# huangjh-pub/di-fusion

Hardware: AMD Instinct MI355X
Metric: frames/s integrate+decode+mesh, 640x480 synthetic stream (higher is better)
Workload: dtype f32

## Files before the change

### di_fusion_amd/_lib.py

```python
from __future__ import annotations

import ctypes
import os
from ctypes import POINTER, Structure, c_float, c_int32, c_int64, c_uint8, c_void_p
from pathlib import Path

PKG = Path(__file__).resolve().parent
LIB_PATH = Path(os.environ["DIF_LIB"]) if os.environ.get("DIF_LIB") else PKG / "libdifusion.so"

C_N_OCCUPIED, C_OVERFLOW, C_ALLOC_NEW, C_M, C_C, C_ITEMS, C_K, C_B, C_VH, C_T, C_QUERY_M, C_N_KEPT, C_CACHE_T, C_CACHE_KEPT, C_EXPORT_N, C_WORK, C_CACHE_DEAD, C_CACHE_LIVE, C_OPT_ROWS, C_OPT_VOXELS, C_HALO_L, C_HALO_R, C_HALO_TICKET, C_DEFERRED = range(24)
C_ALLOC_KEPT = 24
C_STAMP = 31
SYNC_FUSED, SYNC_FRONT_DONE, SYNC_WORDS = 0, 32, 64
FC_COUNT = 32
C_COUNT = 32
PROF_NAMES = ["encode", "decode_lattice", "decode_points", "mc_count", "mc_emit", "halo_export", "halo_merge"]
PROF_COUNT = 8
LATENT_DIM = 29

ERRORS = {-1: "DIF_EINVAL (bad argument)", -2: "DIF_ELAUNCH (HIP launch/runtime failure)", -3: "DIF_ENOSPACE (workspace too small)"}


class DifMap(Structure):
    _fields_ = [("nx", c_int32), ("ny", c_int32), ("nz", c_int32),
# ... 178 lines not shown
    "dif_marching_cubes": (c_int32, [c_void_p, c_int32, c_int32, c_int32, c_void_p, c_int64, c_void_p, c_int64, c_void_p,
                                     c_void_p, c_int32, c_float, c_int64, c_void_p, c_void_p, c_void_p, c_void_p,
                                     c_void_p, c_void_p, c_void_p, c_void_p]),
    "dif_decode_rows": (c_int32, [POINTER(DifWeights), c_void_p, c_int64, c_void_p, c_void_p, c_void_p]),
    "dif_encode_rows": (c_int32, [POINTER(DifWeights), c_void_p, c_int64, c_void_p, c_void_p]),
    "dif_query_sdf": (c_int32, [POINTER(DifMap), POINTER(DifWeights), c_void_p, c_int64, c_void_p, c_void_p, c_void_p,
                                c_void_p, c_void_p, c_void_p, c_void_p]),
    "dif_query_select": (c_int32, [POINTER(DifMap), c_void_p, c_int64, c_void_p, c_void_p, c_void_p, c_void_p, c_int32, c_void_p]),
    "dif_query_decode": (c_int32, [POINTER(DifMap), POINTER(DifWeights), c_void_p, c_int64, c_void_p, c_void_p, c_void_p, c_void_p, c_void_p]),
    "dif_query_grad_scatter": (c_int32, [c_void_p, c_void_p, c_void_p, c_int64, c_void_p, c_void_p]),
    "dif_query_grad_gather": (c_int32, [c_void_p, c_void_p, c_void_p, c_int64, c_void_p, c_void_p]),
    "dif_export_records": (c_int32, [POINTER(DifMap), c_void_p, c_int64, c_int32, c_int32, c_int32, c_void_p, c_void_p]),
    "dif_merge_records": (c_int32, [POINTER(DifMap), c_void_p, c_int64, c_int32, c_void_p, c_void_p]),
    "dif_export_halo": (c_int32, [POINTER(DifMap), c_void_p, c_int64, c_int32, c_int32, c_void_p, c_void_p]),
    "dif_merge_halo": (c_int32, [POINTER(DifMap), c_void_p, c_int64, c_void_p, c_void_p]),
    "dif_export_halo_delta": (c_int32, [POINTER(DifMap), c_void_p, c_void_p, c_int64, c_void_p, c_void_p]),
    "dif_halo_lists_reset": (c_int32, [POINTER(DifMap), c_void_p, c_void_p, c_void_p, c_void_p]),
    "dif_merge_halo2": (c_int32, [POINTER(DifMap), c_void_p, c_int64, c_void_p, c_int64, c_void_p, c_void_p, c_void_p]),
    "dif_profile_enable": (c_int32, [c_int32]),
    "dif_profile_read": (c_int32, [POINTER(ctypes.c_double), POINTER(c_int64), c_int32]),
    "dif_profile_dump": (c_int64, [POINTER(c_int32), POINTER(c_float), c_int64, c_int32]),
    "dif_read_counters": (c_int32, [POINTER(DifMap), POINTER(c_int32), c_void_p]),
    "dif_test_mc_grid_cap": (c_int32, [c_int32]),
    "dif_test_sdma_mode": (c_int32, [c_int32]),
    "dif_test_optimize_views": (c_int32, [c_int64, c_int64, c_void_p, POINTER(DifOptimizeViews)]),
    "dif_test_integrate_views": (c_int32, [c_int64, c_void_p, POINTER(DifIntegrateViews)]),
    "dif_test_sdf_hg_views": (c_int32, [c_int64, c_void_p, POINTER(DifSdfHgViews)]),
    "dif_test_sdf_hg_reduce": (c_int32, [c_void_p, c_int64, POINTER(DifSdfHg), c_void_p, c_int64, c_void_p, c_void_p]),
    "dif_sdma_info": (c_int32, [POINTER(c_int32)]),
    "dif_test_handoff": (c_int32, [c_int32, c_int32, c_int32, c_int32, POINTER(c_int64)]),
    "dif_queues_independent": (c_int32, [c_void_p, c_void_p]),
    "dif_mesh_cache_export_sdma": (c_int32, [POINTER(DifExtractBuffers), c_int64, c_int64, c_void_p, c_void_p, c_void_p]),
    "dif_sdf_hg_workspace_bytes": (c_int64, [c_int64]),
    "dif_sdf_hg": (c_int32, [POINTER(DifMap), POINTER(DifWeights), c_void_p, c_int64, POINTER(DifSdfHg), c_void_p, c_int64, c_void_p, c_void_p,
                             c_int64, c_void_p]),
    "dif_gradient_xy": (c_int32, [c_void_p, c_int32, c_int32, c_void_p, c_void_p]),
    "dif_photo_pyramid": (c_int32, [c_void_p, c_void_p, c_int32, c_int32, POINTER(DifPhotoPyramid), c_void_p]),
    "dif_rgb_odometry": (c_int32, [c_void_p, c_void_p, c_void_p, c_void_p, c_void_p, c_int32, c_int32, POINTER(DifRgbHg), c_void_p, c_void_p,
                                   c_void_p]),
    "dif_rgb_hg_workspace_bytes": (c_int64, []),
    "dif_rgb_hg": (c_int32, [c_void_p, c_void_p, c_void_p, c_void_p, c_void_p, c_int32, c_int32, POINTER(DifRgbHg), c_void_p, c_int64, c_void_p,
                             c_void_p, c_int64, c_void_p]),
}

_lib = None

# ... 63 lines not shown
```

### di_fusion_amd/csrc/difusion.hip

```cpp
#include <cstdlib>
#include <cstdio>
#include <cstring>
#include <mutex>
#include <atomic>
#include <chrono>
#include <vector>
#include <hip/hip_runtime.h>
#include <hsa/hsa.h>
#include <hsa/hsa_ext_amd.h>
#include <dlfcn.h>

#include "common.hip.h"
#include "mlp.hip.h"
#include "mc_tables.inc"

using namespace dif;

namespace {

constexpr int L = DIF_LATENT_DIM;

__device__ __constant__ int c_mc_edge_table[256];
__device__ __constant__ unsigned long long c_mc_tri_packed[256];
bool g_tables_uploaded[64] = {};
// ... 838 lines not shown

struct ExtractGeo { int r, R, l, R3; double sample_a, sample_b; };
static ExtractGeo extract_geo(int resolution) {
    ExtractGeo e;
    e.r = resolution; e.R = 2 * resolution; e.l = resolution;
    e.R3 = e.R * e.R * e.R;
    e.sample_a = -(double)(e.r / 2) * (1.0 / e.r);
    e.sample_b = 1.0 + (double)((e.r - 1) / 2) * (1.0 / e.r);
    return e;
}

static DirtySet dirty_set_of(const dif_map_t* map, const dif_extract_buffers_t* buf, int no_cache) {
    const int64_t grid = (int64_t)map->nx * map->ny * map->nz, plane = (int64_t)map->ny * map->nz;
    const bool tiled = map_is_tiled(map);
    const int64_t own_lo = tiled ? map->own_x_lo * plane : 0, own_hi = tiled ? map->own_x_hi * plane : grid;
    return DirtySet{map->dirty, map->latent_vecs_pos, buf->valid_blocks, map->counters, no_cache, buf->max_voxels, geo_of(map), map->ignore_count_th,
                    map->indexer, map->voxel_obs_count, grid_marks_of(map), own_lo, own_hi, tiled};
}

static VoxelDecodeArgs voxel_decode_args_of(const dif_map_t* map, const dif_weights_t* w, const dif_extract_buffers_t* buf, const ExtractGeo& e, bool fold) {
    VoxelDecodeArgs V = {};
    V.occ_slot = buf->occ_slot; V.latent = map->latent_vecs; V.cube_sdf = buf->cube_sdf; V.cube_std = buf->cube_std;
    V.counters = map->counters;
    V.refine_list = buf->refine_list; V.R = e.R;
    V.fold_w = fold ? w->dec_fold_packed : nullptr; V.fold_table = buf->fold_table;
    V.low.res = e.l; V.low.a = (float)e.sample_a; V.low.vsize = (e.l > 1) ? (float)((e.sample_b - e.sample_a) / (e.l - 1)) : 0.0f;
    return V;
}

static DecodeArgs refine_args_of(const dif_map_t* map, const dif_extract_buffers_t* buf, const ExtractGeo& e, bool fold) {
    DecodeArgs Rf = {};
    Rf.mode = 1; Rf.n_ptr = map->counters + DIF_C_VH; Rf.occ_slot = buf->occ_slot; Rf.latent = map->latent_vecs; Rf.list = buf->refine_list;
    Rf.lat.res = e.R; Rf.lat.a = (float)e.sample_a; Rf.lat.vsize = (float)((e.sample_b - e.sample_a) / (e.R - 1));
    Rf.fold_table = fold ? buf->fold_table : nullptr;
    Rf.out_sdf = buf->cube_sdf; Rf.out_std = buf->cube_std; Rf.sign = -1.0f;
    return Rf;
}

static McArgs mc_args_of(const dif_map_t* map, const dif_extract_buffers_t* buf, const ExtractGeo& e, float max_std, int scale_vertices) {
    int* C = map->counters;
    McArgs a = {};
    a.indexer = map->indexer; a.nx = map->nx; a.ny = map->ny; a.nz = map->nz; a.valid_blocks = buf->valid_blocks; a.K_ptr = C + DIF_C_K; a.K_static = 0;
    a.vbm = map->vbm; a.V = map->capacity; a.cube_sdf = buf->cube_sdf; a.cube_std = buf->cube_std; a.R = e.R; a.max_std = max_std;
    a.max_triangles = buf->cache_capacity; a.new_limit = buf->max_triangles; a.base_ptr = C + DIF_C_CACHE_KEPT;
    a.triangles = buf->cache_tri; a.tri_id = buf->cache_id; a.tri_std = buf->cache_std; a.tri_alive = buf->cache_alive;
    a.scale = scale_vertices ? 1 : 0; a.vs = map->voxel_size; a.bx = map->bound_min[0]; a.by = map->bound_min[1]; a.bz = map->bound_min[2];
    a.log_counters = C;
// ... 24 lines not shown
                                 defer ? (dif_pending_export_t*)map->pending_export : nullptr, buf->stamp, defer ? buf->export_notify : nullptr},
                      (fused_scan && !onepass) ? buf->chunk_sum : nullptr, super_sum, map->dirty_tot, (int)((map->capacity + DIF_BLOCK - 1) / DIF_BLOCK),
                      onepass ? buf->mc_status : nullptr, onepass ? buf->mc_status + (buf->max_voxels + 3) / 4 : nullptr,
                      ov ? map->frame_counters : nullptr};
}

constexpr size_t VD_LDS_F32 = ((size_t)((DEC_LDS_FLOATS + 3) & ~3) + 4 * VD_WAVE_LDS_FLOATS) * 4, VD_LDS_X6 = (size_t)X6_LDS_BYTES + 4 * VD_WAVE_LDS_FLOATS * 4;
static int voxel_decode_attributes() {
    static bool attr_set[64] = {};
    int dev = 0; (void)hipGetDevice(&dev);
    if (dev < 64 && !attr_set[dev]) {
        if (hipFuncSetAttribute((const void*)k_decode_voxels<false>, hipFuncAttributeMaxDynamicSharedMemorySize, (int)VD_LDS_F32) != hipSuccess) return DIF_ELAUNCH;
        if (hipFuncSetAttribute((const void*)k_decode_voxels<true>, hipFuncAttributeMaxDynamicSharedMemorySize, (int)VD_LDS_X6) != hipSuccess) return DIF_ELAUNCH;
        if (hipFuncSetAttribute((const void*)k_decode_refine_x6, hipFuncAttributeMaxDynamicSharedMemorySize, (int)X6_LDS_BYTES) != hipSuccess) return DIF_ELAUNCH;
        if (hipFuncSetAttribute((const void*)k_decode_voxels_batch<true>, hipFuncAttributeMaxDynamicSharedMemorySize, (int)VD_LDS_X6) != hipSuccess) return DIF_ELAUNCH;
        if (hipFuncSetAttribute((const void*)k_decode_refine_x6_batch, hipFuncAttributeMaxDynamicSharedMemorySize, (int)X6_LDS_BYTES) != hipSuccess) return DIF_ELAUNCH;
        attr_set[dev] = true;
    }
    return DIF_OK;
}

static std::atomic<int> g_mc_grid_cap{0};
int dif_test_mc_grid_cap(int32_t n) { return g_mc_grid_cap.exchange(n > 0 ? n : 0); }

static int mc_onepass_setup(const McArgs& a, size_t& lds_bytes, int& grid1, int64_t max_voxels) {
    if (upload_tables() != DIF_OK) return DIF_ELAUNCH;
    const int r = a.R / 2, nc = (r + 1) * (r + 1) * (r + 1);
    lds_bytes = (size_t)(DIF_BLOCK / 64) * MC_ONEPASS_WAVE_LDS_FLOATS(nc) * sizeof(float);
    if (lds_bytes > 128 * 1024) return DIF_EINVAL;
    static bool attr_set1[64] = {};
    int dev = 0; (void)hipGetDevice(&dev);
    if (dev < 64 && !attr_set1[dev]) {
        if (hipFuncSetAttribute((const void*)k_marching_cubes_onepass<0>, hipFuncAttributeMaxDynamicSharedMemorySize, 128 * 1024) != hipSuccess) return DIF_ELAUNCH;
        if (hipFuncSetAttribute((const void*)k_marching_cubes_onepass<4>, hipFuncAttributeMaxDynamicSharedMemorySize, 128 * 1024) != hipSuccess) return DIF_ELAUNCH;
        if (hipFuncSetAttribute((const void*)k_marching_cubes_onepass_batch<0>, hipFuncAttributeMaxDynamicSharedMemorySize, 128 * 1024) != hipSuccess) return DIF_ELAUNCH;
        if (hipFuncSetAttribute((const void*)k_marching_cubes_onepass_batch<4>, hipFuncAttributeMaxDynamicSharedMemorySize, 128 * 1024) != hipSuccess) return DIF_ELAUNCH;
        attr_set1[dev] = true;
    }
    const int64_t need = (max_voxels + 3) / 4;
    int per_cu = (int)((160 * 1024) / (lds_bytes + 1024));
    per_cu = per_cu < 1 ? 1 : per_cu > MC_WAVES_PER_SIMD ? MC_WAVES_PER_SIMD : per_cu;
    grid1 = per_cu * num_cus();
    if (need < grid1) grid1 = (int)(need < 1 ? 1 : need);
    { const int n = g_mc_grid_cap.load(std::memory_order_relaxed); if (n > 0 && n < grid1) grid1 = n; }
    return DIF_OK;
}
// ... 49 lines not shown
    const bool totals = map->dirty_tot && !no_cache && !P.dirty.tiled;
    P.scan = !totals ? DirtyScan::Generic : (map->capacity > 4096 && map->capacity % DIF_BLOCK == 0) ? DirtyScan::BlockTotals : DirtyScan::BoundedTotals;
    if (ov && P.scan != DirtyScan::BlockTotals) return DIF_EINVAL;
    P.fused_word = ov ? map->sync_words + DIF_SYNC_FUSED : nullptr;
    P.grid = (int64_t)map->nx * map->ny * map->nz;
    P.occ = OccFunctor{map->grid_bits, map->indexer, buf->occ_slot, map->vbm, map->counters, max_voxels};

    if (!has_dec(w)) return DIF_EINVAL;
    const bool fused = fast && e.l * e.l * e.l <= VD_MAX_L3 && e.R * e.R <= VD_MAX_R2;
    const bool fold = fused && has_dec_fold(w) && buf->fold_table;
    P.decode = !fast ? DecodeChain::Exact : !fused ? DecodeChain::TwoLevel : (fold && has_dec_x6(w)) ? DecodeChain::FusedX6 : DecodeChain::FusedF32;
    P.refine_tiles = max_voxels * (int64_t)(e.R3 / 32);
    if (P.decode == DecodeChain::Exact) {
        P.lattice = exact_lattice_args_of(map, buf, e);
        P.lattice_tiles = max_voxels * (int64_t)((e.R3 + 31) / 32);
    } else if (P.decode == DecodeChain::TwoLevel) {
        P.lattice = low_lattice_args_of(map, buf, e);
        P.lattice_tiles = max_voxels * ((e.l * e.l * e.l + 31) / 32);
        P.refine = refine_args_of(map, buf, e, false);
    } else {
        P.vd = voxel_decode_args_of(map, w, buf, e, fold);
        if (voxel_decode_attributes() != DIF_OK) return DIF_ELAUNCH;
        P.vd_lds = P.decode == DecodeChain::FusedX6 ? VD_LDS_X6 : VD_LDS_F32;
        P.vd_blocks = cu_blocks(max_voxels, 4);
        P.refine = refine_args_of(map, buf, e, fold);
        P.refine_blocks = cu_blocks(P.refine_tiles, 8);
    }

    P.mc_args = mc_args_of(map, buf, e, max_std, scale_vertices);
    const bool chunked = buf->chunk_sum && max_voxels <= ((int64_t)1 << 24);
    P.mc = !chunked ? McChain::CountScanEmit : (buf->mc_status && e.r * e.r * e.r <= 64) ? McChain::OnePass : McChain::CountEmit;
    int rc = DIF_OK;
    if (P.mc == McChain::OnePass) {
        mc_onepass_args(P.mc_args, map, buf, defer);
        rc = mc_onepass_setup(P.mc_args, P.mc_lds, P.mc_grid, max_voxels);
    } else if (P.mc == McChain::CountEmit) {
        McArgs& a = P.mc_args;
        a.chunk_sum = buf->chunk_sum; a.super_sum = buf->chunk_sum + (max_voxels + 255) / 256; a.tri_start = map->tri_start; a.tri_n = map->tri_n;
        a.tri_count = buf->tri_count; a.tri_offset = nullptr;
        rc = mc_setup(a, P.mc_lds, P.mc_grid, max_voxels);
    }
    if (rc != DIF_OK) return rc;
    P.finish = finish_args_of(map, buf, chunked, P.mc == McChain::OnePass, P.mc_args.out_tri != nullptr, defer);
    P.finish_grid = grid_for(max_voxels, DIF_BLOCK, 256);
    return DIF_OK;
}

// ... 83 lines not shown
    hipStream_t s = (hipStream_t)stream_;
    static thread_local Batch<DirtyScanArgs> dirty; static thread_local ScanBatch<OccFunctor> occ; static thread_local Batch<VoxelDecodeArgs> vd;
    static thread_local Batch<DecodeArgs> rf; static thread_local Batch<McStream> mc; static thread_local Batch<FinishArgs> fin;
    ExtractPlan P;
    for (int j = 0; j < S; ++j) {
        const int rc = extract_plan(st[j].map, w, st[j].buf, resolution, 1, max_std, 0, scale_vertices, s, P);
        if (rc != DIF_OK) return rc;
        if (P.scan != DirtyScan::BlockTotals || P.dirty.tiled || P.decode != DecodeChain::FusedX6 || P.mc != McChain::OnePass) return DIF_EINVAL;
        if (st[j].buf->max_voxels != st[0].buf->max_voxels) return DIF_EINVAL;
        dirty.s[j] = DirtyScanArgs{P.dirty, P.n_slots, st[j].map->dirty_tot};
        occ.f[j] = P.occ; occ.tot[j] = st[j].map->grid_tot;
        vd.s[j] = P.vd; rf.s[j] = P.refine;
        mc.s[j] = McStream{P.mc_args, P.finish.mc_status, P.finish.mc_ticket};
        fin.s[j] = P.finish;
    }
    for (int j = S; j < DIF_MAX_STREAMS; ++j) {
        dirty.s[j] = dirty.s[0]; occ.f[j] = occ.f[0]; occ.tot[j] = occ.tot[0]; vd.s[j] = vd.s[0]; rf.s[j] = rf.s[0]; mc.s[j] = mc.s[0]; fin.s[j] = fin.s[0];
    }
    hipLaunchKernelGGL(k_dirty_scan_batch, dim3((int)(st[0].map->capacity / DIF_BLOCK), S), dim3(DIF_BLOCK), 0, s, dirty);
    DIF_CHECK_LAUNCH();
    if (launch_counted_scan_batch(occ, S, (int)((P.grid + 31) / 32), s) != DIF_OK) return DIF_ELAUNCH;
    {
        ProfScope prof(DIF_PROF_DECODE_LATTICE, s);
        hipLaunchKernelGGL(k_decode_voxels_batch<true>, dim3(cu_blocks(P.occ.max_voxels * S, 4)), dim3(512), P.vd_lds, s, vd, (int)S, (const float*)w->dec_x6_packed);
        DIF_CHECK_LAUNCH();
    }
    {
        ProfScope prof(DIF_PROF_DECODE_POINTS, s);
        hipLaunchKernelGGL(k_decode_refine_x6_batch, dim3(cu_blocks(P.refine_tiles * S, 8)), dim3(512), (size_t)X6_LDS_BYTES, s, rf, (int)S, (const float*)w->dec_x6_packed);
        DIF_CHECK_LAUNCH();
    }
    {
        ProfScope prof(DIF_PROF_MC_COUNT, s);
        if (P.e.r == 4) hipLaunchKernelGGL(k_marching_cubes_onepass_batch<4>, dim3(P.mc_grid, S), dim3(DIF_BLOCK), P.mc_lds, s, mc);
        else hipLaunchKernelGGL(k_marching_cubes_onepass_batch<0>, dim3(P.mc_grid, S), dim3(DIF_BLOCK), P.mc_lds, s, mc);
        DIF_CHECK_LAUNCH();
    }
    hipLaunchKernelGGL(k_extract_finish_batch, dim3(P.finish_grid, S), dim3(DIF_BLOCK), 0, s, fin);
    DIF_CHECK_LAUNCH();
    return DIF_OK;
}

#ifdef DIF_TRACE
int dif_trace_read(unsigned long long* out, int64_t n) {
    return hipMemcpyFromSymbol(out, HIP_SYMBOL(g_vd_trace), (size_t)n * 8) == hipSuccess ? DIF_OK : DIF_ELAUNCH;
}
int dif_trace_read_encode(unsigned long long* out, int64_t n) {
// ... 1294 lines not shown
```

### di_fusion_amd/csrc/kernels_extract.hip.h

```cpp
#pragma once

__device__ __forceinline__ void mark_confident_nbhd(const Geo& g, int lin, float ignore_th, const int64_t* __restrict__ indexer,
                                                    const float* __restrict__ obs, const GridMarks& marks) {
    const uint32_t* bits = marks.bits;
    int ix, iy, iz;
    unlinearize(g, lin, ix, iy, iz);
    int cand[7];
    cand[0] = lin;
    cand[1] = linearize(g, clampi(ix - 1, 0, g.nx - 1), iy, iz);
    cand[2] = linearize(g, clampi(ix + 1, 0, g.nx - 1), iy, iz);
    cand[3] = linearize(g, ix, clampi(iy - 1, 0, g.ny - 1), iz);
    cand[4] = linearize(g, ix, clampi(iy + 1, 0, g.ny - 1), iz);
    cand[5] = linearize(g, ix, iy, clampi(iz - 1, 0, g.nz - 1));
    cand[6] = linearize(g, ix, iy, clampi(iz + 1, 0, g.nz - 1));
    int64_t slot[7];
#pragma unroll
    for (int c = 0; c < 7; ++c) slot[c] = indexer[cand[c]];
    float w[7];
#pragma unroll
    for (int c = 0; c < 7; ++c) w[c] = slot[c] >= 0 ? obs[slot[c]] : ignore_th;
    uint32_t word[7];
#pragma unroll
    for (int c = 0; c < 7; ++c) word[c] = (w[c] > ignore_th) ? bits[cand[c] >> 5] : 0xFFFFFFFFu;
    uint32_t prev[7];
// ... 524 lines not shown
            __syncthreads();
            int o = s_base + ex;
            while (sel) {
                int jz = __ffs((int)sel) - 1;
                sel &= sel - 1;
                refine_list[o++] = (int32_t)(e0 + jz);
            }
        }
        __syncthreads();
    }
}

struct VoxelDecodeArgs {
    const int32_t* occ_slot;
    const float* latent;
    Lattice low;
    int R;
    float* cube_sdf;
    float* cube_std;
    int32_t* refine_list;
    int* counters;
    const float* fold_w;
    float* fold_table;
};

#define VD_MAX_L3 64
#define VD_MAX_R2 64
#define VD_WAVE_LDS_FLOATS (2 * VD_MAX_L3 + 2 * 256)

#ifdef DIF_TRACE
__device__ unsigned long long g_vd_trace[2048 * 8];
#define VD_STAMP(slot) do { if (lane_id() == 0) g_vd_trace[((threadIdx.x >> 6) * gridDim.x + blockIdx.x) * 8 + (slot)] = wall_clock64(); } while (0)
#else
#define VD_STAMP(slot) do { } while (0)
#endif

template <bool X6, int NS>
__device__ __forceinline__ void decode_voxels_body(const BatchN<VoxelDecodeArgs, NS>& AB, int S, const float* __restrict__ wblob) {
    extern __shared__ __attribute__((aligned(16))) float lds[];
    VD_STAMP(0);
    constexpr int LDS_W = X6 ? X6_LDS_BYTES / 4 : ((DEC_LDS_FLOATS + 3) & ~3);
#if defined(DIF_VD_CUT) && DIF_VD_CUT == 0
    return;
#endif
    stage_weights(lds, wblob, X6 ? X6_LDS_BYTES / 4 : DEC_LDS_FLOATS);
    VD_STAMP(1);
#if defined(DIF_VD_CUT) && DIF_VD_CUT == 1
    return;
#endif
    const __amdgpu_buffer_rsrc_t wfwd = make_rsrc(wblob, X6 ? X6_BYTES / 4 : DEC_FLOATS);
    const int lane = lane_id(), half = lane >> 5, col = lane & 31, wid = threadIdx.x >> 6;
    const int pair = wid >> 1, tsel = wid & 1;
    float* w_low_sdf = lds + LDS_W + pair * VD_WAVE_LDS_FLOATS;
    float* w_low_std = w_low_sdf + VD_MAX_L3;
    float* w_fold = w_low_std + VD_MAX_L3 + tsel * 256;
    const Lattice low = AB.s[0].low;
    const float* const fold_w = AB.s[0].fold_w;
    const int l = low.res, R = AB.s[0].R, l3 = l * l * l, R2 = R * R, R3 = R2 * R;
    const float scale = (float)(l - 1) / (float)(R - 1);
    int pre[NS + 1];
    pre[0] = 0;
#pragma unroll
    for (int j = 0; j < NS; ++j) pre[j + 1] = pre[j] + ((j < S) ? AB.s[j].counters[DIF_C_B] : 0);
    const int B = pre[NS];
    const int pairs_per_block = (int)(blockDim.x >> 7), n_pairs = (int)gridDim.x * pairs_per_block;
    const int first = __builtin_amdgcn_readfirstlane(pair * (int)gridDim.x + (int)blockIdx.x);
    __shared__ int s_tot[8], s_map[8], s_base[NS];
    const int rounds = (B + n_pairs - 1) / n_pairs;
    for (int round = 0; round < rounds; ++round) {
        const int bg = first + round * n_pairs;
        int sm = 0, b = bg;
#pragma unroll
        for (int j = 1; j < NS; ++j)
            if (bg >= pre[j]) { sm = j; b = bg - pre[j]; }
        const VoxelDecodeArgs& A = AB.s[sm];
        unsigned sel = 0;
        const int jz0 = tsel * (R >> 1), jz1 = jz0 + (R >> 1);
        const int64_t e0 = (int64_t)b * R3 + (int64_t)lane * R;
        if (bg < B && tsel * 32 < l3) {
            const float* lat_row = A.latent + (int64_t)A.occ_slot[b] * L;
            const int s = tsel * 32 + col;
            const float px = low.coord(s / (l * l)), py = low.coord((s / l) % l), pz = low.coord(s % l);
            float sdf = 0.0f, sd = 0.0f;
            if (X6 || fold_w) {
                if constexpr (X6) decoder_fold_consts_x6(lds, fold_w, lat_row, w_fold, lane);
                else decoder_fold_consts(lds, fold_w, lat_row, w_fold, lane);
                __builtin_amdgcn_wave_barrier();
                __builtin_amdgcn_s_waitcnt(0xc07f);
                if (tsel == 0) {
                    float* rec = A.fold_table + (int64_t)b * 256;
                    for (int p = lane; p < 256; p += 64) rec[p] = w_fold[p];
                }
                VD_STAMP(6);
#if defined(DIF_VD_CUT) && DIF_VD_CUT == 2
                sdf = w_fold[lane]; sd = w_fold[lane + 64];
#else
                if constexpr (X6) decoder_tile_folded_x6(lds, wfwd, FoldInitLds{w_fold}, px, py, pz, lane, sdf, sd);
                else decoder_tile_folded(lds, wfwd, FoldInitLds{w_fold}, px, py, pz, lane, sdf, sd);
#endif
            } else if constexpr (!X6) {
                f16v xin;
#pragma unroll
                for (int t = 0; t < 16; ++t) {
                    const int k = 2 * t + half;
                    xin[t] = (k < L) ? lat_row[k] : 0.0f;
                }
                if (half) { xin[14] = px; xin[15] = pz; } else { xin[15] = py; }
                decoder_tile(lds, wfwd, xin, lane, sdf, sd);
            }
            if (s < l3) {
                if (half == 0) w_low_sdf[s] = sdf;
                else w_low_std[s] = sd;
            }
        }
        __syncthreads();
        VD_STAMP(2);
        if (bg < B && lane < R2) {
            const int jx = lane / R, jy = lane % R;
            int x0, x1, y0, y1; float wx0, wx1, wy0, wy1;
            tri_axis(jx, l, scale, x0, x1, wx0, wx1);
            tri_axis(jy, l, scale, y0, y1, wy0, wy1);
            float* const cube_sdf = A.cube_sdf;
            float* const cube_std = A.cube_std;
            for (int jz = jz0; jz < jz1; ++jz) {
                int z0, z1; float wz0, wz1;
                tri_axis(jz, l, scale, z0, z1, wz0, wz1);
                float sv = tri_sample(w_low_sdf, l, x0, x1, y0, y1, z0, z1, wx0, wx1, wy0, wy1, wz0, wz1);
                float dv = tri_sample(w_low_std, l, x0, x1, y0, y1, z0, z1, wx0, wx1, wy0, wy1, wz0, wz1);
                cube_sdf[e0 + jz] = -sv;
                cube_std[e0 + jz] = dv;
                if (fabsf(sv) < 0.05f) sel |= 1u << jz;
            }
        }
        VD_STAMP(3);
        const int c = __popc(sel);
        const int incl = wave_incl_scan(c);
        const int total = __shfl(incl, 63);
        if (lane == 0) { s_tot[wid] = total; if (NS > 1) s_map[wid] = sm; }
        __syncthreads();
        if (NS == 1) {
            if (threadIdx.x == 0) {
                int sum = 0;
                for (int w = 0; w < (int)(blockDim.x >> 6); ++w) sum += s_tot[w];
                s_base[0] = sum ? atomicAdd(A.counters + DIF_C_VH, sum) : 0;
            }
        } else if ((int)threadIdx.x < S) {
            const int j = (int)threadIdx.x;
            int sum = 0;
            for (int w = 0; w < (int)(blockDim.x >> 6); ++w) sum += (s_map[w] == j) ? s_tot[w] : 0;
            s_base[j] = sum ? atomicAdd(AB.s[j].counters + DIF_C_VH, sum) : 0;
        }
        __syncthreads();
        if (total > 0) {
            int o = s_base[NS == 1 ? 0 : sm] + incl - c;
            for (int w = 0; w < wid; ++w) o += (NS == 1 || s_map[w] == sm) ? s_tot[w] : 0;
            int32_t* const refine_list = A.refine_list;
            while (sel) {
                const int jz = __ffs((int)sel) - 1;
                sel &= sel - 1;
                refine_list[o++] = (int32_t)(e0 + jz);
            }
        }
        __syncthreads();
        VD_STAMP(4);
    }
    VD_STAMP(5);
}

template <bool X6>
__global__ void __launch_bounds__(512, X6 ? 1 : 2) k_decode_voxels(VoxelDecodeArgs A, const float* __restrict__ wblob) {
    const BatchN<VoxelDecodeArgs, 1> B{{A}};
    decode_voxels_body<X6, 1>(B, 1, wblob);
}
template <bool X6>
__global__ void __launch_bounds__(512, X6 ? 1 : 2) k_decode_voxels_batch(Batch<VoxelDecodeArgs> B, int S, const float* __restrict__ wblob) {
    decode_voxels_body<X6, DIF_MAX_STREAMS>(B, S, wblob);
}
```

### di_fusion_amd/csrc/mlp.hip.h

```cpp
#pragma once
#include "common.hip.h"

namespace dif {

typedef float f16v __attribute__((ext_vector_type(16)));
typedef float f4v __attribute__((ext_vector_type(4)));

__device__ __forceinline__ f16v mfma32(float a, float b, f16v c) { return __builtin_amdgcn_mfma_f32_32x32x2f32(a, b, c, 0, 0, 0); }

__device__ __forceinline__ f16v load_bias16(const float* b, int half) {
    const f4v* p = reinterpret_cast<const f4v*>(b + half * 16);
    f4v b0 = p[0], b1 = p[1], b2 = p[2], b3 = p[3];
    f16v r;
    r[0] = b0.x; r[1] = b0.y; r[2] = b0.z; r[3] = b0.w;
    r[4] = b1.x; r[5] = b1.y; r[6] = b1.z; r[7] = b1.w;
    r[8] = b2.x; r[9] = b2.y; r[10] = b2.z; r[11] = b2.w;
    r[12] = b3.x; r[13] = b3.y; r[14] = b3.z; r[15] = b3.w;
    return r;
}

__device__ __forceinline__ float relu1(float x) { return __int_as_float(max(__float_as_int(x), 0)); }
__device__ __forceinline__ f16v relu16(f16v v) {
#pragma unroll
    for (int i = 0; i < 16; ++i) v[i] = relu1(v[i]);
// ... 182 lines not shown

template <int B0, int B3, int UNROLL>
__device__ __forceinline__ void decoder_fold_consts_at(const float* __restrict__ W , const float* __restrict__ fold ,
                                                       const float* __restrict__ lat_row, float* __restrict__ c, int lane) {
    float a0 = W[B0 + lane], a1 = W[B0 + lane + 64], a2 = W[B3 + lane], a3 = W[B3 + lane + 64];
    const f4v* wk = reinterpret_cast<const f4v*>(fold) + lane;
#pragma unroll UNROLL
    for (int k = 0; k < 29; ++k) {
        const float zk = lat_row[k];
        const f4v wv = wk[k * 64];
        a0 = fmaf(wv.x, zk, a0);
        a1 = fmaf(wv.y, zk, a1);
        a2 = fmaf(wv.z, zk, a2);
        a3 = fmaf(wv.w, zk, a3);
    }
    c[lane] = a0;
    c[lane + 64] = a1;
    c[128 + lane] = a2;
    c[128 + lane + 64] = a3;
}
__device__ __forceinline__ void decoder_fold_consts(const float* __restrict__ W, const float* __restrict__ fold, const float* __restrict__ lat_row,
                                                    float* __restrict__ c, int lane) {
    decoder_fold_consts_at<DEC_B0, DEC_B3, 8>(W, fold, lat_row, c, lane);
}

struct FoldInitLds {
    const float* c;
    __device__ __forceinline__ f16v load(int layer, int mb, int half) const { return load_bias16(c + layer * 128 + mb * 32, half); }
};
struct FoldInitGlobal {
    const float* rec;
    __device__ __forceinline__ f16v load(int layer, int mb, int half) const { return load_bias16(rec + layer * 128 + mb * 32, half); }
};

template <class INIT>
__device__ __forceinline__ void decoder_tile_folded(const float* __restrict__ W , __amdgpu_buffer_rsrc_t Wg , const INIT& init,
                                                    float px, float py, float pz, int lane, float& sdf, float& stdv) {
    const int half = lane >> 5;
    const float b14 = half ? px : 0.0f;
    const float b15 = half ? pz : py;
    f16v h0[4];
#pragma unroll
    for (int mb = 0; mb < 4; ++mb) {
        f16v acc = init.load(0, mb, half);
        const f4v a = reinterpret_cast<const f4v*>(W + DEC_A0)[(mb * 4 + 3) * 64 + lane];
        acc = mfma32(a.z, b14, acc);
// ... 722 lines not shown
    f16v g0[4];
#pragma unroll
    for (int mb = 0; mb < 4; ++mb)
        g0[mb] = apply_mask16(block_mm_src<4>(BufA{Wb, offb + DECB_T1 * 4 + mb * 16 * 1024}, g1, zero16(), lane), m0[mb]);
    gx = block_mm_src<4>(BufA{Wb, offb + DECB_T0 * 4}, g0, gskip, lane);
}

__device__ __forceinline__ void stage_weights(float* lds, const float* __restrict__ g, int n_floats) {
    const f4v* __restrict__ src = reinterpret_cast<const f4v*>(g);
    f4v* dst = reinterpret_cast<f4v*>(lds);
    const int n4 = n_floats / 4, step = (int)blockDim.x;
    int i = (int)threadIdx.x;
    for (; i + 7 * step < n4; i += 8 * step) {
        f4v v[8];
#pragma unroll
        for (int k = 0; k < 8; ++k) v[k] = src[i + k * step];
#pragma unroll
        for (int k = 0; k < 8; ++k) dst[i + k * step] = v[k];
    }
    for (; i < n4; i += step) dst[i] = src[i];
    __syncthreads();
}

}
```

### include/difusion.h

```cpp
#ifndef DIFUSION_H
#define DIFUSION_H

#include <stdint.h>

#ifdef __cplusplus
extern "C" {
#endif

#define DIF_VERSION 100
#define DIF_LATENT_DIM 29

#define DIF_MAX_STREAMS 8

#define DIF_OK 0
#define DIF_EINVAL (-1)
#define DIF_ELAUNCH (-2)
#define DIF_ENOSPACE (-3)

enum {
    DIF_C_N_OCCUPIED = 0,
    DIF_C_OVERFLOW = 1,
    DIF_C_ALLOC_NEW = 2,
    DIF_C_M = 3,
    DIF_C_C = 4,
// ... 336 lines not shown
int dif_merge_records(const dif_map_t* map, const int32_t* records, int64_t n, int32_t assign, int32_t* scratch, void* stream);

int dif_export_halo(const dif_map_t* map, int32_t* message, int64_t max_records, int32_t x_lo, int32_t x_hi, int32_t* scratch, void* stream);
int dif_merge_halo(const dif_map_t* map, const int32_t* message, int64_t max_records, int32_t* scratch, void* stream);
int dif_export_halo_delta(const dif_map_t* map, int32_t* msg_left, int32_t* msg_right, int64_t max_records, int32_t* note, void* stream);
int dif_halo_lists_reset(const dif_map_t* map, int32_t* header_left, int32_t* header_right, int32_t* note, void* stream);
int dif_merge_halo2(const dif_map_t* map, const int32_t* msg_a, int64_t max_a, const int32_t* msg_b, int64_t max_b, int32_t* scratch,
                    int32_t* note, void* stream);

enum { DIF_PROF_ENCODE = 0, DIF_PROF_DECODE_LATTICE = 1, DIF_PROF_DECODE_POINTS = 2, DIF_PROF_MC_COUNT = 3, DIF_PROF_MC_EMIT = 4,
       DIF_PROF_HALO_EXPORT = 5 , DIF_PROF_HALO_MERGE = 6 ,
       DIF_PROF_COUNT = 8 };
int dif_profile_enable(int32_t on);
int dif_profile_read(double* ms , int64_t* launches , int32_t reset);
int64_t dif_profile_dump(int32_t* which , float* ms , int64_t capacity, int32_t reset);

int dif_read_counters(const dif_map_t* map, int32_t* host_out , void* stream);

int dif_queues_independent(void* stream_a, void* stream_b);

int dif_mesh_cache_export_sdma(const dif_extract_buffers_t* buf, int64_t lo, int64_t n, float* out_tri, int64_t* out_id, float* out_std);

int dif_test_mc_grid_cap(int32_t n);
int dif_test_sdma_mode(int32_t mode);
typedef struct dif_optimize_views {
    int32_t* row_slot; float* row_xyz; float* row_sdf;
    int32_t* uniq_slot; int32_t* slot_u; int32_t* slot_flag;
    float* z; float* m; float* v;
} dif_optimize_views_t;
int dif_test_optimize_views(int64_t N, int64_t capacity, void* ws, dif_optimize_views_t* out);
typedef struct dif_integrate_views {
    int32_t* pt_lin; uint32_t* pair_list; int32_t* rec_next; int64_t* rec;
} dif_integrate_views_t;
int dif_test_integrate_views(int64_t N, void* ws, dif_integrate_views_t* out);
typedef struct dif_sdf_hg_views {
    float* sdf; float* std; float* grad;
    int64_t partial_offset; int64_t ticket_offset;
} dif_sdf_hg_views_t;
int dif_test_sdf_hg_views(int64_t N, void* ws, dif_sdf_hg_views_t* out);
int dif_test_sdf_hg_reduce(const float* obs_xyz, int64_t N, const dif_sdf_hg_t* args, void* ws, int64_t ws_bytes, double* out, void* stream);
int dif_test_handoff(int32_t mode, int32_t groups, int32_t iters, int32_t flags, int64_t* out);
int dif_sdma_info(int32_t* out);

#ifdef __cplusplus
}
#endif
// ... 2 lines not shown
```

Baseline: 9828.

## Software-pipeline voxel decode: async weight staging, prefetch next latent, deferred list writes

Restructures the voxel-decode kernel so the weight blob is staged into LDS with asynchronous global-to-LDS loads, overlapped with reading counters and the first occupied slot. It prefetches the next round's slot index and latent/fold weights during the current round, and double-buffers shared reservation arrays. Refine-list writes are deferred to the next round, and cube SDF/std stores are buffered in registers and issued after the atomic reservation, which removes one barrier per round. A test hook to cap the decode grid is also added. The cost is higher register pressure and more complex synchronisation; the asynchronous LDS copy is only used on the X6 path.

```diff
diff --git a/di_fusion_amd/_lib.py b/di_fusion_amd/_lib.py
--- a/di_fusion_amd/_lib.py
+++ b/di_fusion_amd/_lib.py
@@ -224,6 +224,7 @@
     "dif_profile_dump": (c_int64, [POINTER(c_int32), POINTER(c_float), c_int64, c_int32]),
     "dif_read_counters": (c_int32, [POINTER(DifMap), POINTER(c_int32), c_void_p]),
     "dif_test_mc_grid_cap": (c_int32, [c_int32]),
+    "dif_test_decode_grid_cap": (c_int32, [c_int32]),
     "dif_test_sdma_mode": (c_int32, [c_int32]),
     "dif_test_optimize_views": (c_int32, [c_int64, c_int64, c_void_p, POINTER(DifOptimizeViews)]),
     "dif_test_integrate_views": (c_int32, [c_int64, c_void_p, POINTER(DifIntegrateViews)]),
diff --git a/di_fusion_amd/csrc/difusion.hip b/di_fusion_amd/csrc/difusion.hip
--- a/di_fusion_amd/csrc/difusion.hip
+++ b/di_fusion_amd/csrc/difusion.hip
@@ -884,7 +884,7 @@
     VoxelDecodeArgs V = {};
     V.occ_slot = buf->occ_slot; V.latent = map->latent_vecs; V.cube_sdf = buf->cube_sdf; V.cube_std = buf->cube_std;
     V.counters = map->counters;
-    V.refine_list = buf->refine_list; V.R = e.R;
+    V.refine_list = buf->refine_list; V.R = e.R; V.max_voxels = (int)(buf->max_voxels < INT32_MAX ? buf->max_voxels : INT32_MAX);
     V.fold_w = fold ? w->dec_fold_packed : nullptr; V.fold_table = buf->fold_table;
     V.low.res = e.l; V.low.a = (float)e.sample_a; V.low.vsize = (e.l > 1) ? (float)((e.sample_b - e.sample_a) / (e.l - 1)) : 0.0f;
     return V;
@@ -955,6 +955,9 @@
 
 static std::atomic<int> g_mc_grid_cap{0};
 int dif_test_mc_grid_cap(int32_t n) { return g_mc_grid_cap.exchange(n > 0 ? n : 0); }
+static std::atomic<int> g_vd_grid_cap{0};
+int dif_test_decode_grid_cap(int32_t n) { return g_vd_grid_cap.exchange(n > 0 ? n : 0); }
+static int vd_grid_capped(int blocks) { const int n = g_vd_grid_cap.load(std::memory_order_relaxed); return (n > 0 && n < blocks) ? n : blocks; }
 
 static int mc_onepass_setup(const McArgs& a, size_t& lds_bytes, int& grid1, int64_t max_voxels) {
     if (upload_tables() != DIF_OK) return DIF_ELAUNCH;
@@ -1050,7 +1053,7 @@
         P.vd = voxel_decode_args_of(map, w, buf, e, fold);
         if (voxel_decode_attributes() != DIF_OK) return DIF_ELAUNCH;
         P.vd_lds = P.decode == DecodeChain::FusedX6 ? VD_LDS_X6 : VD_LDS_F32;
-        P.vd_blocks = cu_blocks(max_voxels, 4);
+        P.vd_blocks = vd_grid_capped(cu_blocks(max_voxels, 4));
         P.refine = refine_args_of(map, buf, e, fold);
         P.refine_blocks = cu_blocks(P.refine_tiles, 8);
     }
@@ -1180,7 +1183,7 @@
     if (launch_counted_scan_batch(occ, S, (int)((P.grid + 31) / 32), s) != DIF_OK) return DIF_ELAUNCH;
     {
         ProfScope prof(DIF_PROF_DECODE_LATTICE, s);
-        hipLaunchKernelGGL(k_decode_voxels_batch<true>, dim3(cu_blocks(P.occ.max_voxels * S, 4)), dim3(512), P.vd_lds, s, vd, (int)S, (const float*)w->dec_x6_packed);
+        hipLaunchKernelGGL(k_decode_voxels_batch<true>, dim3(vd_grid_capped(cu_blocks(P.occ.max_voxels * S, 4))), dim3(512), P.vd_lds, s, vd, (int)S, (const float*)w->dec_x6_packed);
         DIF_CHECK_LAUNCH();
     }
     {
diff --git a/di_fusion_amd/csrc/kernels_extract.hip.h b/di_fusion_amd/csrc/kernels_extract.hip.h
--- a/di_fusion_amd/csrc/kernels_extract.hip.h
+++ b/di_fusion_amd/csrc/kernels_extract.hip.h
@@ -570,10 +570,12 @@
     int* counters;
     const float* fold_w;
     float* fold_table;
+    int max_voxels;
 };
 
 #define VD_MAX_L3 64
 #define VD_MAX_R2 64
+#define VD_MAX_HZ 4
 #define VD_WAVE_LDS_FLOATS (2 * VD_MAX_L3 + 2 * 256)
 
 #ifdef DIF_TRACE
@@ -591,11 +593,7 @@
 #if defined(DIF_VD_CUT) && DIF_VD_CUT == 0
     return;
 #endif
-    stage_weights(lds, wblob, X6 ? X6_LDS_BYTES / 4 : DEC_LDS_FLOATS);
-    VD_STAMP(1);
-#if defined(DIF_VD_CUT) && DIF_VD_CUT == 1
-    return;
-#endif
+    constexpr int W_FLOATS = X6 ? X6_LDS_BYTES / 4 : DEC_LDS_FLOATS;
     const __amdgpu_buffer_rsrc_t wfwd = make_rsrc(wblob, X6 ? X6_BYTES / 4 : DEC_FLOATS);
     const int lane = lane_id(), half = lane >> 5, col = lane & 31, wid = threadIdx.x >> 6;
     const int pair = wid >> 1, tsel = wid & 1;
@@ -606,33 +604,94 @@
     const float* const fold_w = AB.s[0].fold_w;
     const int l = low.res, R = AB.s[0].R, l3 = l * l * l, R2 = R * R, R3 = R2 * R;
     const float scale = (float)(l - 1) / (float)(R - 1);
+    const int pairs_per_block = (int)(blockDim.x >> 7), n_pairs = (int)gridDim.x * pairs_per_block;
+    const int first = __builtin_amdgcn_readfirstlane(pair * (int)gridDim.x + (int)blockIdx.x);
+    int slot_n = AB.s[0].occ_slot[min(first, AB.s[0].max_voxels - 1)];
+    int nb[NS];
+#pragma unroll
+    for (int j = 0; j < NS; ++j) nb[j] = (j < S) ? AB.s[j].counters[DIF_C_B] : 0;
+    __builtin_amdgcn_sched_barrier(0);
+    if constexpr (X6) stage_weights_issue(lds, wblob, W_FLOATS);
+    __builtin_amdgcn_sched_barrier(0);
+#if defined(DIF_VD_CUT) && DIF_VD_CUT == 1
+    if constexpr (X6) stage_weights_wait(); else stage_weights(lds, wblob, W_FLOATS);
+    VD_STAMP(1);
+    return;
+#endif
     int pre[NS + 1];
     pre[0] = 0;
 #pragma unroll
-    for (int j = 0; j < NS; ++j) pre[j + 1] = pre[j] + ((j < S) ? AB.s[j].counters[DIF_C_B] : 0);
+    for (int j = 0; j < NS; ++j) pre[j + 1] = pre[j] + nb[j];
     const int B = pre[NS];
-    const int pairs_per_block = (int)(blockDim.x >> 7), n_pairs = (int)gridDim.x * pairs_per_block;
-    const int first = __builtin_amdgcn_readfirstlane(pair * (int)gridDim.x + (int)blockIdx.x);
-    __shared__ int s_tot[8], s_map[8], s_base[NS];
-    const int rounds = (B + n_pairs - 1) / n_pairs;
-    for (int round = 0; round < rounds; ++round) {
-        const int bg = first + round * n_pairs;
-        int sm = 0, b = bg;
+    auto locate = [&](int bg, int& sm, int& b) {
+        sm = 0; b = bg;
 #pragma unroll
         for (int j = 1; j < NS; ++j)
             if (bg >= pre[j]) { sm = j; b = bg - pre[j]; }
+    };
+    if (NS > 1 && first >= pre[1]) {
+        slot_n = 0;
+        if (first < B) { int sm0, b0; locate(first, sm0, b0); slot_n = AB.s[sm0].occ_slot[b0]; }
+    }
+    __shared__ int s_tot[2][8], s_map[2][8], s_base[2][NS];
+    const int rounds = (B + n_pairs - 1) / n_pairs;
+    if (rounds == 0) {
+        if constexpr (X6) stage_weights_wait();
+        return;
+    }
+    const int hz = R >> 1, jz0 = tsel * hz;
+    const bool folded = X6 || fold_w;
+    const __amdgpu_buffer_rsrc_t wfold = make_rsrc(fold_w, folded ? DECF_FLOATS : 0);
+    unsigned sel_p = 0; int e0_p = 0, off_p = 0, sm_p = 0;
+    int vzero = 0;
+    asm volatile("" : "+v"(vzero));
+    auto write_list = [&](int par) {
+        if (sel_p) {
+            int o = s_base[par][NS == 1 ? 0 : sm_p] + off_p;
+            int32_t* const refine_list = AB.s[sm_p].refine_list;
+            while (sel_p) {
+                const int jz = __ffs((int)sel_p) - 1;
+                sel_p &= sel_p - 1;
+                refine_list[o++] = (int32_t)(e0_p + jz);
+            }
+        }
+    };
+    float zl = 0.0f;
+    f4v w0[X6 ? 15 : 8];
+    auto request_fold_inputs = [&](int bgq, int slot) {
+        zl = 0.0f;
+        if (folded && bgq < B && tsel * 32 < l3) {
+            int smq, bq;
+            locate(bgq, smq, bq);
+            const float* lat = AB.s[smq].latent + (int64_t)slot * L;
+            zl = lat[lane < L ? lane : L - 1];
+        }
+        decoder_fold_w_first(wfold, lane, w0);
+    };
+    request_fold_inputs(first, slot_n);
+    if constexpr (X6) stage_weights_wait();
+    else stage_weights(lds, wblob, W_FLOATS);
+    VD_STAMP(1);
+    for (int round = 0; round < rounds; ++round) {
+        const int par = round & 1;
+        const int bg = first + round * n_pairs;
+        int sm, b;
+        locate(bg, sm, b);
         const VoxelDecodeArgs& A = AB.s[sm];
-        unsigned sel = 0;
-        const int jz0 = tsel * (R >> 1), jz1 = jz0 + (R >> 1);
-        const int64_t e0 = (int64_t)b * R3 + (int64_t)lane * R;
-        if (bg < B && tsel * 32 < l3) {
-            const float* lat_row = A.latent + (int64_t)A.occ_slot[b] * L;
+        const bool live = bg < B, tile = live && tsel * 32 < l3;
+        const float* lat_row = A.latent + (int64_t)(tile ? slot_n : 0) * L;
+        {
+            const int bgn = bg + n_pairs;
+            slot_n = 0;
+            if (bgn < B) { int smn, bn; locate(bgn, smn, bn); slot_n = AB.s[smn].occ_slot[bn + vzero]; }
+        }
+        if (tile) {
             const int s = tsel * 32 + col;
             const float px = low.coord(s / (l * l)), py = low.coord((s / l) % l), pz = low.coord(s % l);
             float sdf = 0.0f, sd = 0.0f;
-            if (X6 || fold_w) {
-                if constexpr (X6) decoder_fold_consts_x6(lds, fold_w, lat_row, w_fold, lane);
-                else decoder_fold_consts(lds, fold_w, lat_row, w_fold, lane);
+            if (folded) {
+                if constexpr (X6) decoder_fold_consts_pre<X6_B0, X6_B3, 15>(lds, wfold, zl, w0, w_fold, lane);
+                else decoder_fold_consts_pre<DEC_B0, DEC_B3, 8>(lds, wfold, zl, w0, w_fold, lane);
                 __builtin_amdgcn_wave_barrier();
                 __builtin_amdgcn_s_waitcnt(0xc07f);
                 if (tsel == 0) {
@@ -643,8 +702,10 @@
 #if defined(DIF_VD_CUT) && DIF_VD_CUT == 2
                 sdf = w_fold[lane]; sd = w_fold[lane + 64];
 #else
-                if constexpr (X6) decoder_tile_folded_x6(lds, wfwd, FoldInitLds{w_fold}, px, py, pz, lane, sdf, sd);
-                else decoder_tile_folded(lds, wfwd, FoldInitLds{w_fold}, px, py, pz, lane, sdf, sd);
+                int lane_t = lane;
+                asm volatile("" : "+v"(lane_t));
+                if constexpr (X6) decoder_tile_folded_x6(lds, wfwd, FoldInitLds{w_fold}, px, py, pz, lane_t, sdf, sd);
+                else decoder_tile_folded(lds, wfwd, FoldInitLds{w_fold}, px, py, pz, lane_t, sdf, sd);
 #endif
             } else if constexpr (!X6) {
                 f16v xin;
@@ -663,55 +724,63 @@
         }
         __syncthreads();
         VD_STAMP(2);
-        if (bg < B && lane < R2) {
-            const int jx = lane / R, jy = lane % R;
+        write_list(par ^ 1);
+        const bool up = live && lane < R2;
+        const int e0 = up ? b * R3 + lane * R : 0;
+        unsigned sel = 0;
+        float cs[VD_MAX_HZ], cd[VD_MAX_HZ];
+        if (up) {
+            int lane_r = lane;
+            int jz0_r = jz0;
+            asm volatile("" : "+v"(lane_r), "+v"(jz0_r));
+            const int jx = lane_r / R, jy = lane_r % R;
             int x0, x1, y0, y1; float wx0, wx1, wy0, wy1;
             tri_axis(jx, l, scale, x0, x1, wx0, wx1);
             tri_axis(jy, l, scale, y0, y1, wy0, wy1);
-            float* const cube_sdf = A.cube_sdf;
-            float* const cube_std = A.cube_std;
-            for (int jz = jz0; jz < jz1; ++jz) {
-                int z0, z1; float wz0, wz1;
-                tri_axis(jz, l, scale, z0, z1, wz0, wz1);
-                float sv = tri_sample(w_low_sdf, l, x0, x1, y0, y1, z0, z1, wx0, wx1, wy0, wy1, wz0, wz1);
-                float dv = tri_sample(w_low_std, l, x0, x1, y0, y1, z0, z1, wx0, wx1, wy0, wy1, wz0, wz1);
-                cube_sdf[e0 + jz] = -sv;
-                cube_std[e0 + jz] = dv;
-                if (fabsf(sv) < 0.05f) sel |= 1u << jz;
+#pragma unroll
+            for (int t = 0; t < VD_MAX_HZ; ++t) {
+                if (t < hz) {
+                    const int jz = jz0_r + t;
+                    int z0, z1; float wz0, wz1;
+                    tri_axis(jz, l, scale, z0, z1, wz0, wz1);
+                    const float sv = tri_sample(w_low_sdf, l, x0, x1, y0, y1, z0, z1, wx0, wx1, wy0, wy1, wz0, wz1);
+                    const float dv = tri_sample(w_low_std, l, x0, x1, y0, y1, z0, z1, wx0, wx1, wy0, wy1, wz0, wz1);
+                    cs[t] = -sv;
+                    cd[t] = dv;
+                    if (fabsf(sv) < 0.05f) sel |= 1u << jz;
+                }
             }
         }
         VD_STAMP(3);
         const int c = __popc(sel);
         const int incl = wave_incl_scan(c);
         const int total = __shfl(incl, 63);
-        if (lane == 0) { s_tot[wid] = total; if (NS > 1) s_map[wid] = sm; }
+        if (lane == 0) { s_tot[par][wid] = total; if (NS > 1) s_map[par][wid] = sm; }
         __syncthreads();
-        if (NS == 1) {
-            if (threadIdx.x == 0) {
-                int sum = 0;
-                for (int w = 0; w < (int)(blockDim.x >> 6); ++w) sum += s_tot[w];
-                s_base[0] = sum ? atomicAdd(A.counters + DIF_C_VH, sum) : 0;
-            }
-        } else if ((int)threadIdx.x < S) {
-            const int j = (int)threadIdx.x;
+        const bool reserves = (NS == 1) ? threadIdx.x == 0 : (int)threadIdx.x < S;
+        int got = 0;
+        if (reserves) {
+            const int j = (NS == 1) ? 0 : (int)threadIdx.x;
             int sum = 0;
-            for (int w = 0; w < (int)(blockDim.x >> 6); ++w) sum += (s_map[w] == j) ? s_tot[w] : 0;
-            s_base[j] = sum ? atomicAdd(AB.s[j].counters + DIF_C_VH, sum) : 0;
-        }
-        __syncthreads();
-        if (total > 0) {
-            int o = s_base[NS == 1 ? 0 : sm] + incl - c;
-            for (int w = 0; w < wid; ++w) o += (NS == 1 || s_map[w] == sm) ? s_tot[w] : 0;
-            int32_t* const refine_list = A.refine_list;
-            while (sel) {
-                const int jz = __ffs((int)sel) - 1;
-                sel &= sel - 1;
-                refine_list[o++] = (int32_t)(e0 + jz);
-            }
-        }
-        __syncthreads();
+            for (int w = 0; w < (int)(blockDim.x >> 6); ++w) sum += (NS == 1 || s_map[par][w] == j) ? s_tot[par][w] : 0;
+            if (sum) got = atomicAdd(AB.s[j].counters + DIF_C_VH, sum);
+        }
+        if (up) {
+            float* const cube_sdf = A.cube_sdf + e0 + jz0;
+            float* const cube_std = A.cube_std + e0 + jz0;
+#pragma unroll
+            for (int t = 0; t < VD_MAX_HZ; ++t)
+                if (t < hz) { cube_sdf[t] = cs[t]; cube_std[t] = cd[t]; }
+        }
+        if (reserves) s_base[par][(NS == 1) ? 0 : (int)threadIdx.x] = got;
+        int off = incl - c;
+        for (int w = 0; w < wid; ++w) off += (NS == 1 || s_map[par][w] == sm) ? s_tot[par][w] : 0;
+        sel_p = sel; e0_p = e0; off_p = off; sm_p = sm;
+        request_fold_inputs(bg + n_pairs, slot_n);
         VD_STAMP(4);
     }
+    __syncthreads();
+    write_list((rounds - 1) & 1);
     VD_STAMP(5);
 }
 
diff --git a/di_fusion_amd/csrc/mlp.hip.h b/di_fusion_amd/csrc/mlp.hip.h
--- a/di_fusion_amd/csrc/mlp.hip.h
+++ b/di_fusion_amd/csrc/mlp.hip.h
@@ -228,6 +228,47 @@
 __device__ __forceinline__ void decoder_fold_consts(const float* __restrict__ W, const float* __restrict__ fold, const float* __restrict__ lat_row,
                                                     float* __restrict__ c, int lane) {
     decoder_fold_consts_at<DEC_B0, DEC_B3, 8>(W, fold, lat_row, c, lane);
+}
+
+template <int UNROLL>
+__device__ __forceinline__ void decoder_fold_w_first(__amdgpu_buffer_rsrc_t fold, int lane, f4v (&w0)[UNROLL]) {
+    const BufA wk{fold, 0};
+#pragma unroll
+    for (int k = 0; k < UNROLL; ++k) w0[k] = wk.load(k, lane);
+}
+template <int B0, int B3, int UNROLL>
+__device__ __forceinline__ void decoder_fold_consts_pre(const float* __restrict__ W , __amdgpu_buffer_rsrc_t fold ,
+                                                        float zl, const f4v (&w0)[UNROLL], float* __restrict__ c, int lane) {
+    auto z = [&](int k) { return __builtin_bit_cast(float, __builtin_amdgcn_readlane(__builtin_bit_cast(int, zl), k)); };
+    float a0 = W[B0 + lane], a1 = W[B0 + lane + 64], a2 = W[B3 + lane], a3 = W[B3 + lane + 64];
+    const BufA wk{fold, 0};
+#pragma unroll
+    for (int k = 0; k < UNROLL; ++k) {
+        const float zk = z(k);
+        a0 = fmaf(w0[k].x, zk, a0);
+        a1 = fmaf(w0[k].y, zk, a1);
+        a2 = fmaf(w0[k].z, zk, a2);
+        a3 = fmaf(w0[k].w, zk, a3);
+    }
+#pragma unroll
+    for (int k0 = UNROLL; k0 < 29; k0 += UNROLL) {
+        __builtin_amdgcn_sched_barrier(0);
+        f4v wv[UNROLL];
+#pragma unroll
+        for (int k = k0; k < k0 + UNROLL && k < 29; ++k) wv[k - k0] = wk.load(k, lane);
+#pragma unroll
+        for (int k = k0; k < k0 + UNROLL && k < 29; ++k) {
+            const float zk = z(k);
+            a0 = fmaf(wv[k - k0].x, zk, a0);
+            a1 = fmaf(wv[k - k0].y, zk, a1);
+            a2 = fmaf(wv[k - k0].z, zk, a2);
+            a3 = fmaf(wv[k - k0].w, zk, a3);
+        }
+    }
+    c[lane] = a0;
+    c[lane + 64] = a1;
+    c[128 + lane] = a2;
+    c[128 + lane + 64] = a3;
 }
 
 struct FoldInitLds {
@@ -996,4 +1037,18 @@
     __syncthreads();
 }
 
-}
+__device__ __forceinline__ void stage_weights_issue(float* lds, const float* __restrict__ g, int n_floats) {
+    typedef __attribute__((address_space(1))) const void* gptr_t;
+    typedef __attribute__((address_space(3))) void* lptr_t;
+    const f4v* src = reinterpret_cast<const f4v*>(g);
+    f4v* dst = reinterpret_cast<f4v*>(lds);
+    const int n4 = n_floats / 4, lane = (int)(threadIdx.x & 63), step = (int)blockDim.x;
+    for (int c = __builtin_amdgcn_readfirstlane((int)(threadIdx.x & ~63u)); c < n4; c += step)
+        if (c + lane < n4) __builtin_amdgcn_global_load_lds((gptr_t)(src + c + lane), (lptr_t)(dst + c), 16, 0, 0);
+}
+__device__ __forceinline__ void stage_weights_wait() {
+    __builtin_amdgcn_s_waitcnt(0x0f70);
+    __syncthreads();
+}
+
+}
diff --git a/include/difusion.h b/include/difusion.h
--- a/include/difusion.h
+++ b/include/difusion.h
@@ -382,6 +382,7 @@
 int dif_mesh_cache_export_sdma(const dif_extract_buffers_t* buf, int64_t lo, int64_t n, float* out_tri, int64_t* out_id, float* out_std);
 
 int dif_test_mc_grid_cap(int32_t n);
+int dif_test_decode_grid_cap(int32_t n);
 int dif_test_sdma_mode(int32_t mode);
 typedef struct dif_optimize_views {
     int32_t* row_slot; float* row_xyz; float* row_sdf;
```

New measurement: 8932. -9.1%, worse.
